# fxslava/tiny_mp2v_dec

Hardware: AMD Instinct MI355X
Metric: decoded frames/sec + GB/s vs HBM roofline, 1080p 4:2:0 @1/2/4/8 GPU; bit-exact YUV (higher is better)
Workload: dtype u8

## Files before the change

### tiny_mp2v_dec_amd/csrc/recon.hip

```cpp
#include <hip/hip_runtime.h>

#include <cstdlib>
#include <stdint.h>
#include <stdlib.h>

#include "recon_kernel.h"

namespace mp2vg {

typedef short short2_t __attribute__((ext_vector_type(2)));

__device__ __forceinline__ short2_t adds2(short2_t a, short2_t b) { return __builtin_elementwise_add_sat(a, b); }
__device__ __forceinline__ short2_t subs2(short2_t a, short2_t b) { return __builtin_elementwise_sub_sat(a, b); }
__device__ __forceinline__ short2_t shl2(short2_t a, int n) {
    return __builtin_bit_cast(short2_t, __builtin_bit_cast(ushort2, a) << (unsigned short)n);
}
__device__ __forceinline__ short2_t mulhi2(short2_t a, int c) {
    const uint32_t u = __builtin_bit_cast(uint32_t, a);
    const int lo = (int)(short)(u & 0xffffu) * c, hi = ((int)u >> 16) * c;
    return __builtin_bit_cast(short2_t, __builtin_amdgcn_perm((uint32_t)hi, (uint32_t)lo, 0x07060302u));
}
__device__ __forceinline__ short2_t mulhi2_x2(short2_t a, int c) {
    const short2_t h = mulhi2(a, 2 * c);
    return __builtin_bit_cast(short2_t, __builtin_bit_cast(uint32_t, h) & 0xfffefffeu);
// ... 137 lines not shown
    static constexpr int SIZE = 256 + 2 * F::CW * F::CH;
#ifndef MP2VG_RES_PAD
#define MP2VG_RES_PAD 0
#endif
    static constexpr int MBS = SIZE + MP2VG_RES_PAD;
    __device__ static constexpr int base(int plane) { return plane == 0 ? 0 : 256 + (plane - 1) * F::CW * F::CH; }
    __device__ static constexpr int width(int plane) { return plane == 0 ? 16 : F::CW; }
    __device__ static int pos(int x) { return (x & ~3) | ((x & 1) << 1) | ((x >> 1) & 1); }
};

template <class T>
__device__ __forceinline__ T gsel(const T (&v)[3], int plane) {
    return plane == 0 ? v[0] : (plane == 1 ? v[1] : v[2]);
}

#ifndef MP2VG_REC_NT
#define MP2VG_REC_NT 0
#endif
__device__ __forceinline__ uint32_t ld_rec(const uint32_t* p) {
    if (MP2VG_REC_NT) return __builtin_nontemporal_load(p);
    return *p;
}
__device__ __forceinline__ uint32_t rec_load(const uint32_t* __restrict__ mbrec, uint32_t g, uint32_t mb_last, int lane) {
    const uint32_t mb = min(g + (uint32_t)(lane & 3), mb_last);
    return ld_rec(&mbrec[(size_t)mb * 8 + ((lane >> 2) & 7)]);
}
__device__ __forceinline__ uint32_t rec_get(uint32_t rv, int f, int k) {
    return (uint32_t)__builtin_amdgcn_ds_bpermute((f * 4 + k) * 4, (int)rv);
}
template <int F, int K>
// ... 17 lines not shown

template <int NB, int K>
__device__ __forceinline__ void group_mb(Group& S, uint32_t rv, int ng, int& sb, int& cr) {
    const uint32_t r1 = rec_uni<1, K>(rv), r2 = rec_uni<2, K>(rv);
    const bool live = K < ng;
    const uint32_t cbpk = live ? ((r1 >> 16) & ((1u << NB) - 1)) : 0u;
    S.fl8 |= (live ? (r1 & 0xff) : (uint32_t)MP2VG_MB_INTRA) << (8 * K);
    S.qs8 |= (r2 & 0xff) << (8 * K);
    S.sb8 |= (uint32_t)sb << (8 * K);
    if (K == 0) S.cbp01 = cbpk;
    if (K == 1) S.cbp01 |= cbpk << 16;
    if (K == 2) S.cbp23 = cbpk;
    if (K == 3) S.cbp23 |= cbpk << 16;
    sb += __builtin_popcount(cbpk);
    cr += live ? (int)(r2 >> 16) : 0;
}

template <int NB>
__device__ __forceinline__ Group group_state(uint32_t rv, int ng) {
    Group S;
    S.fl8 = S.qs8 = S.sb8 = 0;
    int sb = 0, cr = 0;
    group_mb<NB, 0>(S, rv, ng, sb, cr);
    group_mb<NB, 1>(S, rv, ng, sb, cr);
    group_mb<NB, 2>(S, rv, ng, sb, cr);
    group_mb<NB, 3>(S, rv, ng, sb, cr);
    S.nslots = sb;
    S.ncoef = cr;
    S.coef0 = rec_uni<3, 0>(rv);
    return S;
// ... 177 lines not shown
};
__device__ __forceinline__ LaneRec lane_rec(uint32_t rv, int lane) {
    LaneRec L;
    const int k = lane & 3;
    L.r0 = rec_get(rv, 0, k);
    L.r1 = rec_get(rv, 1, k);
    const int r = (L.r1 & MP2VG_MB_FIELD_MC) ? ((lane >> 2) & 1) : 0;
    L.mvf = rec_get(rv, 4 + 2 * r, k);
    L.mvb = rec_get(rv, 5 + 2 * r, k);
    return L;
}

template <int CF, int MCM, int J, int NW, int ABL = 0>
__device__ __forceinline__ void issue_pass(const LaneRec& L, bool live, int lane, const Geo& geo,
                                           __amdgpu_buffer_rsrc_t ref_fwd, __amdgpu_buffer_rsrc_t ref_bwd,
                                           Tap<NW>& tf, Tap<NW>& tb, int dir = 0) {
    using F = Fmt<CF>;
    int k, plane, py;
    pass_row<CF, J>(lane, k, plane, py);
    const uint32_t fl = L.r1 & 0xffff;
    const bool none = !live || (fl & MP2VG_MB_INTRA);
    const bool bwd = fl & MP2VG_MB_BWD;
    const bool fwd = !none && (MCM == 1 || (fl & MP2VG_MB_FWD) || !bwd);
    const bool field = fl & MP2VG_MB_FIELD_MC;
    const int pw = plane == 0 ? 16 : F::CW;
    const int phm = plane == 0 ? 16 : F::CH;
    const int gx = (int)(L.r0 & 0xffff) * pw;
    const int mbyb = (int)(L.r0 >> 16) * phm;
    const int r = field ? (py & 1) : 0;
    const int stride = J == 0 ? geo.stride[0] : geo.stride[1];
    const int ph = J == 0 ? geo.ph[0] : geo.ph[1];
    constexpr bool TL = J == 0 || kChromaTiles;
    const uint32_t off = (TL ? 2u : 1u) * (uint32_t)gsel(geo.plane_off, plane);
    const uint32_t mv1 = (MCM == 1 && dir) ? L.mvb : L.mvf;
    const int fsh = 8 + 2 * r + (MCM == 1 ? dir : 0);
    constexpr bool R2 = MP2VG_ROW2_LOAD && MCM == 2;
    tap_issue<CF, NW, ABL, TL, R2>(tf, fwd, ref_fwd, off, mv1, plane, gx, py, phm, mbyb, field, (fl >> fsh) & 1, stride, ph);
    if (MCM == 2)
        tap_issue<CF, NW, ABL, TL, R2>(tb, !none && bwd, ref_bwd, off, L.mvb, plane, gx, py, phm, mbyb, field,
                                       (fl >> (9 + 2 * r)) & 1, stride, ph);
}

__device__ __forceinline__ void row_store16(uint8_t* d, uint32_t a, uint32_t b, uint32_t c, uint32_t e) {
    *(uint4*)d = make_uint4(a, b, c, e);
}
// ... 41 lines not shown
            const uint4 q1 = *(const uint4*)&res[8];
            rv[4] = q1.x; rv[5] = q1.y; rv[6] = q1.z; rv[7] = q1.w;
        }
#pragma unroll
        for (int d = 0; d < NW; d++) {
            if (!(d < 2 ? cl : cr)) continue;
            const uint32_t lo = __builtin_amdgcn_perm(0u, out[d], 0x0c020c00u);
            const uint32_t hi = __builtin_amdgcn_perm(0u, out[d], 0x0c030c01u);
            const short2_t a = __builtin_bit_cast(short2_t, lo) + __builtin_bit_cast(short2_t, rv[2 * d]);
            const short2_t c = __builtin_bit_cast(short2_t, hi) + __builtin_bit_cast(short2_t, rv[2 * d + 1]);
            out[d] = __builtin_amdgcn_perm(sat_pk_u8(c), sat_pk_u8(a), 0x05010400u);
        }
    }
    const int pw = plane == 0 ? 16 : F::CW;
    const int phm = plane == 0 ? 16 : F::CH;
    const uint32_t doff = gsel(geo.plane_off, plane) + mul24_asm((r0 >> 16) * phm + py, (uint32_t)gsel(geo.stride, plane)) +
                          (r0 & 0xffff) * (uint32_t)pw;
    uint8_t* dst = dst_slot + doff;
    dst = live ? dst : wsink;
    if (ABL & 8192)
        dst = dst_slot + ((((r0 & 0xffff) + (r0 >> 16) * 128u) * 3u + (uint32_t)J) * 1024u + (uint32_t)lane * 16u) %
                             (uint32_t)(geo.plane_off[1] - 1024);
    if (tiles) {
        uint8_t* img = (uint8_t*)(s_res_wave + k * RL::MBS + RL::base(plane) + py * RL::width(plane));
        if (NW == 4)
            *(uint4*)img = make_uint4(out[0], out[1], out[2], out[3]);
        else
            *(uint2*)img = make_uint2(out[0], out[1]);
    }
    if (ABL & 8) {
        asm volatile("" ::"v"(out[0]), "v"(out[1]), "v"(out[2]), "v"(out[3]), "v"(dst));
// ... 11 lines not shown
        row_store8(dst, out[0], out[1]);
    }
}

template <int CF, int J, int NW>
__device__ __forceinline__ void store_pass_put8(uint32_t r0, bool live, int lane, const Geo& geo, uint8_t* wsink,
                                                uint8_t* dst_slot, __amdgpu_buffer_rsrc_t dst_rsrc,
                                                const uint8_t* res8_wave) {
    using F = Fmt<CF>;
    using RL = ResLayout<CF>;
    int k, plane, py;
    pass_row<CF, J>(lane, k, plane, py);
    const uint8_t* row = &res8_wave[k * RL::SIZE + RL::base(plane) + py * RL::width(plane)];
    const int pw = plane == 0 ? 16 : F::CW;
    const int phm = plane == 0 ? 16 : F::CH;
    const uint32_t doff = gsel(geo.plane_off, plane) + mul24_asm((r0 >> 16) * phm + py, (uint32_t)gsel(geo.stride, plane)) +
                          (r0 & 0xffff) * (uint32_t)pw;
    uint8_t* dst = live ? dst_slot + doff : wsink;
    if (NW == 4) {
        const uint4 q = *(const uint4*)row;
        const uint4 o = make_uint4(__builtin_amdgcn_perm(q.x, q.x, 0x03010200u), __builtin_amdgcn_perm(q.y, q.y, 0x03010200u),
                                   __builtin_amdgcn_perm(q.z, q.z, 0x03010200u), __builtin_amdgcn_perm(q.w, q.w, 0x03010200u));
        if (MP2VG_ROW_POL != 0)
            pol_store16<MP2VG_ROW_POL>(dst_rsrc, live ? doff : kNoTap, o);
        else
            row_store16(dst, o.x, o.y, o.z, o.w);
    } else {
        const uint2 q = *(const uint2*)row;
        const uint2 o = make_uint2(__builtin_amdgcn_perm(q.x, q.x, 0x03010200u), __builtin_amdgcn_perm(q.y, q.y, 0x03010200u));
        if (MP2VG_ROW_POL != 0)
            pol_store8<MP2VG_ROW_POL>(dst_rsrc, live ? doff : kNoTap, o);
// ... 13 lines not shown
    const uint4 q = *(const uint4*)img_row<CF, NAT>(img, k, plane, py);
    return make_uint4(unswz(q.x, NAT), unswz(q.y, NAT), unswz(q.z, NAT), unswz(q.w, NAT));
}
template <int CF, bool NAT>
__device__ __forceinline__ uint2 img_row8(const uint8_t* img, int k, int plane, int py) {
    const uint2 q = *(const uint2*)img_row<CF, NAT>(img, k, plane, py);
    return make_uint2(unswz(q.x, NAT), unswz(q.y, NAT));
}
template <int CF, bool NAT, int ABL = 0>
__device__ __forceinline__ void tile_group(uint32_t mx0, uint32_t mby, int lane, const Geo& geo, uint8_t* wsink,
                                           uint8_t* dst_tiles, __amdgpu_buffer_rsrc_t tile_rsrc, const uint8_t* res8) {
    using F = Fmt<CF>;
    constexpr bool POL = MP2VG_TILE_POL != 0;
    for (int plane = 0; plane < (CF == 3 && kChromaTiles ? 3 : 1); plane++) {
        uint8_t* tp = dst_tiles + 2u * gsel(geo.plane_off, plane);
        const uint32_t ncol = (uint32_t)gsel(geo.stride, plane) >> 4;
#pragma nounroll
        for (int i = 0; i < 2; i++) {
            const int u = lane + 64 * i;
            int j, r, h;
            if (u < 96) {
                j = u >> 5, r = ((u >> 3) & 3) * 4 + ((u & 7) >> 1), h = u & 1;
            } else {
                const int side = (u - 96) >> 4;
                r = u & 15, h = side, j = side ? -1 : 3;
            }
            const uint4 v = img_row16<CF, NAT>(res8, j + h, plane, r);
            const bool none = j < 0 && mx0 == 0;
            const uint32_t o = tile_row<16>(mx0 + (uint32_t)j, mby * 16u + (uint32_t)r, ncol) + (uint32_t)h * 16u;
            if (POL)
                pol_store16<MP2VG_TILE_POL>(tile_rsrc, none ? kNoTap : 2u * gsel(geo.plane_off, plane) + o, v);
// ... 116 lines not shown
        pa = (lds_uint4_t*)(uintptr_t)(b0 + (uint32_t)(ca << 4));
        pb = (lds_uint4_t*)(uintptr_t)(b0 + (uint32_t)(cb << 4));
    }
}
__device__ __forceinline__ void put8_rows(uint32_t a0, uint32_t step, const short2_t (&s)[8]) {
#pragma unroll
    for (int y = 0; y < 8; y++) *(lds_u16_t*)(uintptr_t)(a0 + (uint32_t)y * step) = (uint16_t)sat_pk_u8(s[y] >> (short)6);
}

struct SliceCtx {
    const uint32_t* mbrec;
    const uint32_t* coefs;
    uint8_t* dst_slot;
    uint8_t* dst_tiles;
    __amdgpu_buffer_rsrc_t dst_rsrc, tile_rsrc;
    bool tiles;
    int dir;
    uint8_t* wsink;
    __amdgpu_buffer_rsrc_t ref_fwd, ref_bwd;
    __amdgpu_buffer_rsrc_t cref_fwd, cref_bwd;
    __amdgpu_buffer_rsrc_t coef_rsrc;
    uint32_t mb_begin, mb_end;
    uint32_t wpos, step;
    int half;
};

template <int CF>
__device__ __forceinline__ uint32_t dq_entry(const Group& S, int lane) {
    constexpr int NB = Fmt<CF>::NB;
    const int k = lane >> 4, bb = lane & 15;
    const uint32_t cbpk = pick16(S.cbp01, S.cbp23, k);
    const bool coded = bb < NB && ((cbpk >> bb) & 1);
    const uint32_t slot = pick8(S.sb8, k) + (uint32_t)__builtin_popcount(cbpk & ((1u << bb) - 1));
    const uint32_t intra = pick8(S.fl8, k) & MP2VG_MB_INTRA;
    const uint32_t wsel = (bb < 6 ? 0u : 2u) + (intra ? 0u : 1u);
    return (slot & 0xff) | (pick8(S.qs8, k) << 8) | (wsel << 16) | (intra << 18) | ((uint32_t)coded << 19);
}

__device__ __forceinline__ int mul24i_asm(int a, int b) {
    int r;
    asm("v_mul_i32_i24 %0, %1, %2" : "=v"(r) : "v"(a), "v"(b));
    return r;
}

template <class LT, bool INTRA_ONLY = false, int NB = 6>
__device__ __forceinline__ void dequant_word(LT& L, int wave, uint32_t w, uint32_t qs8, bool live = true, int h = 0,
                                             int buf = 0) {
    if constexpr (INTRA_ONLY) {
        const uint32_t k = (w >> 26) & 3u, b = (w >> 22) & 15u;
        const int slot = (int)(k * NB + b);
// ... 102 lines not shown
    if (g >= mb_end) return;
    const int kl = lane & 3;

    Tap<4> t0f, t0b;
    Tap<NWC> t1f, t1b;
    Tap<NWC> t2f, t2b;
    Group S;
    constexpr int NCW = MCM == 0 ? (CF == 3 ? 24 : (CF == 2 ? 12 : 8)) : 2;
    uint32_t gr0, gr1, rvN, cw[NCW];
    bool glive;
    {
        const uint32_t rv = rec_load(c.mbrec, g, mb_last, lane);
        const int ng = (int)min(mb_end - g, (uint32_t)G);
        glive = kl < ng;
        const LaneRec R = lane_rec(rv, lane);
        if (MCM) issue_pass<CF, MCM, 0, 4, ABL>(R, glive, lane, geo, c.ref_fwd, c.ref_bwd, t0f, t0b, c.dir);
        S = group_state<NB>(rv, ng);
        gr0 = R.r0;
        gr1 = R.r1;
        __builtin_amdgcn_sched_barrier(0);
        rvN = rec_load(c.mbrec, g + STEP < mb_end ? g + STEP : g, mb_last, lane);
        prefetch_words<MCM, NCW>(cw, c, S.coef0, S.ncoef, lane);
        __builtin_amdgcn_sched_barrier(0);
        if (MCM) {
            issue_pass<CF, MCM, 1, NWC, ABL>(R, glive, lane, geo, c.cref_fwd, c.cref_bwd, t1f, t1b, c.dir);
            if (CF != 1) issue_pass<CF, MCM, 2, NWC, ABL>(R, glive, lane, geo, c.cref_fwd, c.cref_bwd, t2f, t2b, c.dir);
        }
        __builtin_amdgcn_sched_barrier(0);
        if (!(ABL & 8)) {
#pragma unroll
            for (int j = 0; j < Passes<CF>::N; j++) ((uint32_t*)c.wsink)[j * 4] = 0u;
        }
    }

    Stamps st;
#pragma unroll
    for (int i = 0; i < 7; i++) st.acc[i] = 0;
    stamp<ABL>(st, -1);
    for (; g < mb_end; g += STEP) {
        stamp<ABL>(st, 6);
        uint32_t p0[4] = {0, 0, 0, 0}, p1[NWC], p2[NWC];
// ... 2 lines not shown
        if (MCM) {
            touch(t0f), touch(t1f);
            if (MCM == 2) touch(t0b), touch(t1b);
            if (CF != 1) touch(t2f);
            if (CF != 1 && MCM == 2) touch(t2b);
            predict<MCM, 4, ABL>(t0f, t0b, lane, p0);
            predict<MCM, NWC, ABL>(t1f, t1b, lane, p1);
            if (CF != 1) predict<MCM, NWC, ABL>(t2f, t2b, lane, p2);
        }

        stamp<ABL>(st, 0);
        const uint32_t gn = g + STEP < mb_end ? g + STEP : g;
        const int ngN = (int)min(mb_end - gn, (uint32_t)G);
        const bool gliveN = kl < ngN;
        const LaneRec R = lane_rec(rvN, lane);
        if (MCM) issue_pass<CF, MCM, 0, 4, ABL>(R, gliveN, lane, geo, c.ref_fwd, c.ref_bwd, t0f, t0b, c.dir);
        const Group SN = group_state<NB>(rvN, ngN);
        __builtin_amdgcn_sched_barrier(0);
        rvN = rec_load(c.mbrec, g + 2 * STEP < mb_end ? g + 2 * STEP : g, mb_last, lane);

        stamp<ABL>(st, 1);
        if constexpr (MCM != 0) {
            const uint32_t e = dq_entry<CF>(S, lane);
            L.dq[wave][lane] = e;
            if (e & (1u << 19)) L.map[wave][e & 0xff] = (uint8_t)lane;
            wave_sync();
        }
        if (!(ABL & 4)) {
            if constexpr (MCM == 0) {
#pragma unroll
                for (int j = 0; j < NCW; j++) {
                    if (64 * j >= S.ncoef) break;
                    dequant_word<LT, true, NB>(L, wave, cw[j], S.qs8, 64 * j + lane < S.ncoef, c.half);
                }
            } else {
#pragma unroll
                for (int j = 0; j < NCW; j++)
                    if (64 * j + lane < S.ncoef) dequant_word<LT, false, NB>(L, wave, cw[j], S.qs8, true, c.half);
            }
            constexpr int XW = MCM == 0 ? 8 : 2;
// ... 34 lines not shown
                if (v == 0 && intra) par ^= ra.x & 1u;
                par = (par ^ (par >> 16)) & 1u;
                par ^= (uint32_t)__builtin_amdgcn_ds_swizzle((int)par, 0x041F);
                par ^= (uint32_t)__builtin_amdgcn_ds_swizzle((int)par, 0x081F);
                if (v == 6) rb.w ^= (par ^ 1u) << 16;
                short2_t s[8] = {__builtin_bit_cast(short2_t, ra.x), __builtin_bit_cast(short2_t, ra.y),
                                 __builtin_bit_cast(short2_t, ra.z), __builtin_bit_cast(short2_t, ra.w),
                                 __builtin_bit_cast(short2_t, rb.x), __builtin_bit_cast(short2_t, rb.y),
                                 __builtin_bit_cast(short2_t, rb.z), __builtin_bit_cast(short2_t, rb.w)};
                idct_1d<true>(s);
                pass1_store<LT>(bw, slot, v, s);
            }
            wave_sync();
            __builtin_amdgcn_sched_barrier(0);
            if (MCM) {
                issue_pass<CF, MCM, 1, NWC, ABL>(R, gliveN, lane, geo, c.cref_fwd, c.cref_bwd, t1f, t1b, c.dir);
                if (CF != 1) issue_pass<CF, MCM, 2, NWC, ABL>(R, gliveN, lane, geo, c.cref_fwd, c.cref_bwd, t2f, t2b, c.dir);
            }
            __builtin_amdgcn_sched_barrier(0);
            stamp<ABL>(st, 3);
            for (int t = lane; t < (((ABL & 1) || ((ABL & (131072 | 262144)) && odd)) ? 0 : S.nslots * 4); t += 64) {
                const int slot = t >> 2, xq = t & 3;
                const int x = (xq & 1) | ((xq & 2) << 1);
                short* const bw = (short*)L.blk[wave];
                lds_uint4_t *pa, *pb;
                slot_chunks<LT>(bw, slot, x, x + 2, pa, pb);
                const uint4 ra = ld16(pa);
                const uint4 rb = ld16(pb);
                zero16(pa);
                zero16(pb);
                short2_t s[8];
                interleave(ra, rb, s);
// ... 64 lines not shown
                        int plane, x0, y0, ys;
                        block_origin<CF>(bb, dctf, plane, x0, y0, ys);
                        const int rw = RL::width(plane);
                        const int xp = RL::pos(x0 + x);
                        const uint32_t a0 = (uint32_t)(uintptr_t)(lds_u16_t*)((uint8_t*)L.res[wave] + RL::base(plane)) +
                                            mul24_asm((uint32_t)k, (uint32_t)RL::SIZE) + (uint32_t)(y0 * rw + xp);
                        put8_rows(a0, (uint32_t)(ys * rw), sv);
                    }
                }
                wave_sync();
            }
            stamp<ABL>(st, 3);
        }

        stamp<ABL>(st, 4);
        if constexpr (LT::COMPACT) {
            const uint8_t* res8 = (const uint8_t*)L.res[wave];
            store_pass_put8<CF, 0, 4>(gr0, glive, lane, geo, c.wsink, c.dst_slot, c.dst_rsrc, res8);
            store_pass_put8<CF, 1, NWC>(gr0, glive, lane, geo, c.wsink, c.dst_slot, c.dst_rsrc, res8);
            if (CF != 1) store_pass_put8<CF, 2, NWC>(gr0, glive, lane, geo, c.wsink, c.dst_slot, c.dst_rsrc, res8);
            if (TILES && c.tiles) {
                const uint32_t r00 = (uint32_t)__builtin_amdgcn_readfirstlane((int)gr0);
                tile_group<CF, false, ABL>(r00 & 0xffff, r00 >> 16, lane, geo, c.wsink, c.dst_tiles, c.tile_rsrc, res8);
            }
        } else {
            store_pass<CF, 0, 4, ABL>(gr0, gr1, glive, lane, geo, c.wsink, c.dst_slot, c.dst_rsrc, MCM != 2 && c.tiles, L.res[wave], p0);
            store_pass<CF, 1, NWC, ABL>(gr0, gr1, glive, lane, geo, c.wsink, c.dst_slot, c.dst_rsrc, MCM != 2 && c.tiles, L.res[wave], p1);
            if (CF != 1) store_pass<CF, 2, NWC, ABL>(gr0, gr1, glive, lane, geo, c.wsink, c.dst_slot, c.dst_rsrc, MCM != 2 && c.tiles, L.res[wave], p2);
            if (MCM != 2 && c.tiles) {
                wave_sync();
                const uint32_t r00 = (uint32_t)__builtin_amdgcn_readfirstlane((int)gr0);
                tile_group<CF, true, ABL>(r00 & 0xffff, r00 >> 16, lane, geo, c.wsink, c.dst_tiles, c.tile_rsrc,
                                          (const uint8_t*)L.res[wave]);
            }
        }
        wave_sync();

        stamp<ABL>(st, 5);
        S = SN;
        gr0 = R.r0;
        gr1 = R.r1;
        glive = gliveN;
    }
    if ((ABL & 16) && lane == 0) {
        unsigned long long* out = (unsigned long long*)(geo.sink + 1024) + 8 * MCM;
#pragma unroll
        for (int i = 0; i < 7; i++) atomicAdd(&out[i], (unsigned long long)st.acc[i]);
        atomicAdd(&out[7], 1ull);
    }
}

template <int CF, int MCM, int ABL = 0>
__global__ __launch_bounds__((64 * kernel_waves<MCM, ABL>())) __attribute__((amdgpu_waves_per_eu((MCM == 0 || MCM == 4) && (ABL & ~kAblCompact) == 0 ? (CF == 3 ? 4 : 6) : (CF == 3 ? 3 : 4)))) void recon_kernel(const mp2vg_picture_t* __restrict__ pics,
                                                    const uint32_t* __restrict__ mbrec,
                                                    const uint32_t* __restrict__ coefs,
                                                    const SliceDesc* __restrict__ slices,
                                                    const Geo geo,
                                                    const uint32_t slice_base, const uint32_t nslices,
                                                    const uint32_t mates) {
    using LT = Lds<CF, compact_layout<MCM, ABL>(), kernel_waves<MCM, ABL>()>;
    __shared__ __attribute__((aligned(128))) LT L;
    const int tid = threadIdx.x;
    const int lane = tid & 63;
    const int wave = __builtin_amdgcn_readfirstlane(tid >> 6);
    static_assert(slices_per_wg<CF, MCM, ABL>(4) <= (uint32_t)LT::NH, "one matrix set per slice");
    const uint32_t spw = slices_per_wg<CF, MCM, ABL>(mates);
    const bool two = spw > 1;
    const uint32_t wps = 4u / spw;
    const uint32_t nunits = (nslices + spw - 1) / spw;
    const uint32_t b = blockIdx.x, q8 = nunits / 8, r8 = nunits % 8, xcd = b % 8;
    const uint32_t unit = xcd * q8 + min(xcd, r8) + b / 8;
    const int half = two ? (int)((uint32_t)wave / wps) : 0;
    const uint32_t si = spw * unit + (uint32_t)half;
    const bool have = si < nslices;
    const SliceDesc sd = slices[slice_base + min(si, nslices - 1)];
    const mp2vg_picture_t* pic = pics + sd.pic;
// ... 6 lines not shown
        L.scan[64 * half + lane] = (uint8_t)(LT::WB ? 2 * pos : pos);
        if constexpr (LT::WB && MP2VG_I_KBTAB) {
            const int k = lane >> 4, bb = lane & 15;
            const uint32_t slot = (uint32_t)(k * Fmt<CF>::NB + (bb < Fmt<CF>::NB ? bb : 0));
            L.kbtab[lane] = (((slot << 7) | ((slot << 4) & 0x70u)) << 8) | ((uint32_t)k * 8u);
        }
        if constexpr (LT::WB && CF != 1) {
#pragma unroll
            for (int bb = 0; bb < Fmt<CF>::NB; bb++) L.Wb[bb][lane] = pic->W[bb < 6 ? 0 : 2][lane];
        }
    }
    for (int i = lane; i < LT::NBUF * LT::MAXS * LT::BLK / 2; i += 64) ((uint32_t*)L.blk[wave * LT::NBUF])[i] = 0;
    __syncthreads();
    if (!have) return;

    SliceCtx c;
    c.mbrec = mbrec;
    c.coefs = coefs;
    c.dst_slot = (uint8_t*)geo.ftab[pic->dst_slot];
    c.wsink = geo.sink + 2048 + ((b * LT::NWAVES + wave) & 1023) * 64;
    c.dst_tiles = (uint8_t*)geo.ttab[pic->dst_slot];
    c.dst_rsrc = slot_rsrc(c.dst_slot, (uint32_t)geo.slot_bytes);
    c.tile_rsrc = slot_rsrc(c.dst_tiles, (uint32_t)(2 * geo.slot_bytes));
    c.tiles = sd.reserved & 1u;
    const bool one_dir = sd.reserved & 2u;
    c.dir = (sd.reserved >> 2) & 1u;
    const int fs0 = pic->fwd_slot < 0 ? pic->dst_slot : pic->fwd_slot;
    const int bs = pic->bwd_slot < 0 ? pic->dst_slot : pic->bwd_slot;
    const int fs = c.dir ? bs : fs0;
    c.ref_fwd = slot_rsrc((const uint8_t*)geo.ttab[fs], (uint32_t)(2 * geo.slot_bytes));
    c.ref_bwd = slot_rsrc((const uint8_t*)geo.ttab[bs], (uint32_t)(2 * geo.slot_bytes));
    if (kChromaTiles) {
        c.cref_fwd = c.ref_fwd, c.cref_bwd = c.ref_bwd;
    } else {
        c.cref_fwd = slot_rsrc((const uint8_t*)geo.ftab[fs], (uint32_t)geo.slot_bytes);
        c.cref_bwd = slot_rsrc((const uint8_t*)geo.ftab[bs], (uint32_t)geo.slot_bytes);
    }
    c.coef_rsrc = __builtin_amdgcn_make_buffer_rsrc((void*)coefs, (short)0, (int)kNoTap, 0x00020000);
    c.mb_begin = sd.mb_begin;
    c.mb_end = sd.mb_begin + sd.mb_count;
    c.half = half;
    c.wpos = two ? (uint32_t)wave % wps : (uint32_t)wave;
    c.step = (two ? wps : (uint32_t)LT::NWAVES) * G;
    if constexpr (MCM == 4) {
        run_slice<CF, 0, ABL, LT, false>(c, geo, L, lane, wave);
    } else if constexpr (MCM < 3) {
        run_slice<CF, (ABL & 2) ? 0 : MCM, ABL, LT>(c, geo, L, lane, wave);
    } else {
        const int pct = pic->picture_coding_type;
        if (pct == 3 && !one_dir)
            run_slice<CF, (ABL & 2) ? 0 : 2, ABL, LT>(c, geo, L, lane, wave);
        else if (pct == 2 || one_dir)
            run_slice<CF, (ABL & 2) ? 0 : 1, ABL, LT>(c, geo, L, lane, wave);
        else
            run_slice<CF, 0, ABL, LT>(c, geo, L, lane, wave);
    }
}
__device__ __forceinline__ uint64_t mix64(uint64_t z) {
    z = (z ^ (z >> 30)) * 0xBF58476D1CE4E5B9ull;
    z = (z ^ (z >> 27)) * 0x94D049BB133111EBull;
    return z ^ (z >> 31);
}

__global__ void digest_kernel(const uint64_t* __restrict__ ftab, const int32_t* __restrict__ slots,
                              uint64_t o0, uint64_t o1, uint64_t o2, int s0, int s1, int w0, int w1, int h0, int h1,
                              unsigned long long* __restrict__ out) {
    const int si = blockIdx.y;
    const uint8_t* base = (const uint8_t*)ftab[slots[si]];
    const int rows = h0 + 2 * h1;
    uint64_t acc = 0;
    for (int row = blockIdx.x; row < rows; row += gridDim.x) {
// ... 9 lines not shown
            p = base + o2 + (uint64_t)(row - h0 - h1) * s1;
            w = w1;
        }
        for (int x = threadIdx.x * 4; x < w; x += blockDim.x * 4) {
            const uint32_t d = *(const uint32_t*)(p + x);
            acc += mix64(mix64(((uint64_t)row << 32) | (uint64_t)x) ^ (uint64_t)d);
        }
    }
    for (int off = 32; off > 0; off >>= 1) acc += __shfl_xor(acc, off);
    if ((threadIdx.x & 63) == 0) atomicAdd(&out[si], (unsigned long long)acc);
}

template <int CF, int MCM, int ABL>
static void launch_one(const KArgs& a, const Geo& g, hipStream_t stream) {
    const uint32_t spw = slices_per_wg<CF, MCM, ABL>(a.mates);
    hipLaunchKernelGGL((recon_kernel<CF, MCM, ABL>), dim3((a.nslices + spw - 1) / spw),
                       dim3(64 * kernel_waves<MCM, ABL>()), 0, stream, a.pics, (const uint32_t*)a.mbs, a.coefs,
                       a.slices, g, a.slice_base, a.nslices, spw);
}

template <int CF, int ABL>
static hipError_t launch_mcm(int mcm, const KArgs& a, const Geo& g, hipStream_t stream) {
    switch (mcm) {
    case 0: launch_one<CF, 0, ABL>(a, g, stream); break;
    case 1: launch_one<CF, 1, ABL>(a, g, stream); break;
    case 2: launch_one<CF, 2, ABL>(a, g, stream); break;
    case 3: launch_one<CF, 3, ABL>(a, g, stream); break;
    case 4: launch_one<CF, 4, ABL>(a, g, stream); break;
    default: return hipErrorInvalidValue;
    }
    return hipGetLastError();
}

hipError_t launch_recon(int cf, int mcm, const KArgs& a, hipStream_t stream) {
    Geo g;
    g.sink = a.sink;
    g.slot_bytes = a.slot_bytes;
    g.ftab = a.ftab;
    g.ttab = a.ttab;
    for (int i = 0; i < 3; i++) {
        g.plane_off[i] = (uint32_t)a.plane_off[i];
        g.stride[i] = a.stride[i];
        g.ph[i] = a.ph[i];
    }
    static const int ablate = getenv("MP2VG_ABLATE") ? atoi(getenv("MP2VG_ABLATE")) : 0;
#ifndef MP2VG_DEV_ABLATIONS
    if (ablate) return hipErrorNotSupported;
#else
    if (cf == 3 && ablate == 16) return launch_mcm<3, 16>(mcm, a, g, stream);
    if (cf == 1 && ablate) {
        switch (ablate) {
        case 1: return launch_mcm<1, 1>(mcm, a, g, stream);
        case 2: return launch_mcm<1, 2>(mcm, a, g, stream);
        case 4: return launch_mcm<1, 4>(mcm, a, g, stream);
        case 8: return launch_mcm<1, 8>(mcm, a, g, stream);
        case 15: return launch_mcm<1, 15>(mcm, a, g, stream);
        case 16: return launch_mcm<1, 16>(mcm, a, g, stream);
        case 32: return launch_mcm<1, 32>(mcm, a, g, stream);
        case 64: return launch_mcm<1, 64>(mcm, a, g, stream);
// ... 205 lines not shown
```

### tiny_mp2v_dec_amd/csrc/recon_kernel.h

```cpp
#pragma once
#include <hip/hip_runtime.h>
#include <stdint.h>

#include "../../include/mp2vg.h"

namespace mp2vg {

struct SliceDesc {
    uint32_t pic;
    uint32_t mb_begin;
    uint32_t mb_count;
    uint32_t reserved;
};

struct Launch {
    uint32_t begin, end;
    int mcm;
    int mates = 0;
    int level;
    int set;
};

struct Geo {
    uint8_t* sink;
    uint64_t slot_bytes;
    const uint64_t* ftab;
    const uint64_t* ttab;
    uint32_t plane_off[3];
    int32_t stride[3];
    int32_t ph[3];
};

struct KArgs {
    const mp2vg_picture_t* pics;
    const mp2vg_mb_t* mbs;
    const uint32_t* coefs;
    const SliceDesc* slices;
    uint8_t* sink;
    uint64_t slot_bytes;
    const uint64_t *ftab, *ttab;
    uint64_t plane_off[3];
    int32_t stride[3];
    int32_t ph[3];
    uint32_t slice_base;
    uint32_t nslices;
    uint32_t mates = 0;
};

constexpr int kFrameCopyMax = 32;
struct FrameCopy {
    const uint8_t* src[kFrameCopyMax];
    uint8_t* dst[kFrameCopyMax];
};
hipError_t launch_frame_copy(const FrameCopy& fc, int n, uint64_t bytes, hipStream_t stream);

}
```

### tiny_mp2v_dec_amd/csrc/runtime.cpp

```cpp
#include <hip/hip_runtime.h>

#include <algorithm>
#include <cstdio>
#include <cstring>
#include <string>
#include <vector>
#include <atomic>
#include <thread>

#include "export_kernel.h"
#include "hipchk.h"
#include "recon_kernel.h"
#include "syntax.h"

namespace mp2vg {
hipError_t launch_recon(int cf, int mcm, const KArgs& a, hipStream_t stream);
hipError_t launch_tile_convert(const KArgs& a, int cf, const int32_t* d_list, int n, int32_t slot0, hipStream_t stream);
hipError_t launch_clock_probe(unsigned long long* d_out, int iters, int blocks, hipStream_t stream);
hipError_t launch_block_probe(void* p, size_t bytes, int rw, int reps, void* sink, hipStream_t stream);
hipError_t launch_block_random(const void* base, size_t bytes, int waves, int iters, void* sink, hipStream_t stream);
hipError_t launch_pool_scatter(const uint64_t* tab, int nslots, uint32_t fkb, uint32_t tkb, int lock, int waves,
                               int iters, void* sink, hipStream_t stream);
hipError_t launch_digest(const uint64_t* ftab, const int32_t* d_slots, int n,
                         const uint64_t off[3], const int32_t stride[3], const int32_t w[3],
// ... 701 lines not shown
            } else if (types == 1 && slice_rows == 1 && i_split > 1 && (mbw / i_split) % 4 == 0 && mbw % i_split == 0) {
                const int pw = mbw / i_split;
                for (int r = 0; r < mbh; r++)
                    for (size_t k = i; k < j; k++)
                        for (int q = 0; q < i_split; q++)
                            slices.push_back({(uint32_t)lp[k], pics[lp[k]].mb_first + (uint32_t)(r * mbw + q * pw),
                                              (uint32_t)pw, sflags(lp[k])});
            } else {
                for (int r = 0; r < mbh; r += slice_rows)
                    for (size_t k = i; k < j; k++) push(k, r);
            }
            i = j;
        }
        l.end = (uint32_t)slices.size();
        l.mcm = types == 1 ? 0 : (types == 2 ? 1 : (types == 4 ? 2 : 3));
        static const int tilefree = dev_env("MP2VG_I_TILEFREE") ? atoi(dev_env("MP2VG_I_TILEFREE")) : 0;
        int nneed = 0;
        for (int p : lp) nneed += need[p];
        if (types == 1 && (tilefree == 2 || (tilefree && c->g.cf != 3 && nneed * 4 <= (int)lp.size()))) {
            l.mcm = 4;
            for (uint32_t k = l.begin; k < l.end; k++) slices[k].reserved = 0;
        }
        l.level = q;
        l.set = set;
        l.mates = (mates && types != 1 && l.mcm != 0 && l.mcm != 4 && mbw % 4 == 0) ? (c->g.cf == 3 ? std::min(mates, 2) : mates) : 0;
        if (tplan)
            for (int p : lp)
                if (need[p] && (pics[p].picture_coding_type == 3 || l.mcm == 4))
                    tplan->post.push_back({(int32_t)launches.size(), pics[p].dst_slot});
        launches.push_back(l);
// ... 372 lines not shown
        for (int set = 0; set < nsets; set++) {
            const int i = launch_at(set, k);
            if (i < 0) continue;
            const hipStream_t st = stream_of(set);
            if (couple == 1 && nsets > 1) {
                for (int t = 0; t < nsets; t++)
                    if (t != set && launch_at(t, k - 1) >= 0) HIPCHK(hipStreamWaitEvent(st, c->lev[launch_at(t, k - 1)], 0));
            } else if (couple == 2 && nsets > 1) {
                if (set > 0 && launch_at(set - 1, k) >= 0) HIPCHK(hipStreamWaitEvent(st, c->lev[launch_at(set - 1, k)], 0));
                if (set + 1 < nsets && launch_at(set + 1, k - 2) >= 0)
                    HIPCHK(hipStreamWaitEvent(st, c->lev[launch_at(set + 1, k - 2)], 0));
            }
            a.slice_base = launches[i].begin;
            a.nslices = launches[i].end - launches[i].begin;
            a.mates = (uint32_t)launches[i].mates;
            if (c->launch_timing) HIPCHK(hipEventRecord(H.l[2 * i], st));
            if (a.nslices) HIPCHK(launch_recon(c->g.cf, launches[i].mcm, a, st));
            {
                const auto r = b.post_of[i];
                if (r.second > r.first)
                    HIPCHK(launch_tile_convert(a, c->g.cf, b.d_post + r.first, r.second - r.first, 0, st));
            }
            if (c->launch_timing) HIPCHK(hipEventRecord(H.l[2 * i + 1], st));
            if (couple && nsets > 1) HIPCHK(hipEventRecord(c->lev[i], st));
        }
    for (int set = 0; set < nsets; set++) {
        HIPCHK(hipEventRecord(c->sev[set], stream_of(set)));
        HIPCHK(hipStreamWaitEvent(c->stream, c->sev[set], 0));
    }
    c->last_foot.assign(nsets, std::vector<uint8_t>(c->nslots, 0));
// ... 376 lines not shown
```

Measured before the change: 385,100.

## Split mixed-launch kernel by intra presence and cut scalar register pressure

Adds a separate mixed-type recon kernel that is used only when a launch contains I pictures, so the common mixed P/B kernel no longer instantiates the intra loop body. Uses asm-based rematerialization tricks (fresh_s, reloading kernel args per loop instantiation, readfirstlane for uniform bases) to keep strides, pointers and flags in SGPRs instead of holding them live across the loop. Splits group state computation into early/late parts to shorten live ranges, and simplifies dq_entry bit extraction. The intent is lower register pressure and smaller code, at the cost of extra scalar reloads and more kernel variants.

```diff
diff --git a/tiny_mp2v_dec_amd/csrc/recon.hip b/tiny_mp2v_dec_amd/csrc/recon.hip
--- a/tiny_mp2v_dec_amd/csrc/recon.hip
+++ b/tiny_mp2v_dec_amd/csrc/recon.hip
@@ -1,6 +1,8 @@
 #include <hip/hip_runtime.h>
 
+#include <cstddef>
 #include <cstdlib>
+#include <type_traits>
 #include <stdint.h>
 #include <stdlib.h>
 
@@ -175,6 +177,16 @@
     return plane == 0 ? v[0] : (plane == 1 ? v[1] : v[2]);
 }
 
+template <class T>
+__device__ __forceinline__ T fresh_s(T v, uint32_t tick) {
+    asm("" : "+s"(v) : "s"(tick));
+    return v;
+}
+
+__device__ __forceinline__ int32_t plane_stride(const Geo& geo, int plane) {
+    return plane == 0 ? geo.stride[0] : geo.stride[1];
+}
+
 #ifndef MP2VG_REC_NT
 #define MP2VG_REC_NT 0
 #endif
@@ -222,6 +234,48 @@
     if (K == 3) S.cbp23 |= cbpk << 16;
     sb += __builtin_popcount(cbpk);
     cr += live ? (int)(r2 >> 16) : 0;
+}
+
+struct GroupEarly {
+    uint32_t qs8;
+    int ncoef;
+    uint32_t coef0;
+};
+__device__ __forceinline__ GroupEarly group_early(uint32_t rv, int ng) {
+    GroupEarly E;
+    const uint32_t r2[4] = {rec_uni<2, 0>(rv), rec_uni<2, 1>(rv), rec_uni<2, 2>(rv), rec_uni<2, 3>(rv)};
+    E.qs8 = 0;
+    E.ncoef = 0;
+#pragma unroll
+    for (int k = 0; k < 4; k++) {
+        E.qs8 |= (r2[k] & 0xff) << (8 * k);
+        E.ncoef += k < ng ? (int)(r2[k] >> 16) : 0;
+    }
+    E.coef0 = rec_uni<3, 0>(rv);
+    return E;
+}
+template <int NB>
+__device__ __forceinline__ Group group_late(const GroupEarly& E, uint32_t r1_lanes, int ng) {
+    Group S;
+    S.fl8 = S.sb8 = 0;
+    S.cbp01 = S.cbp23 = 0;
+    int sb = 0;
+#pragma unroll
+    for (int k = 0; k < 4; k++) {
+        const uint32_t r1 = (uint32_t)__builtin_amdgcn_readlane((int)r1_lanes, k);
+        const bool live = k < ng;
+        const uint32_t cbpk = live ? ((r1 >> 16) & ((1u << NB) - 1)) : 0u;
+        S.fl8 |= (live ? (r1 & 0xff) : (uint32_t)MP2VG_MB_INTRA) << (8 * k);
+        S.sb8 |= (uint32_t)sb << (8 * k);
+        if (k < 2) S.cbp01 |= cbpk << (16 * k);
+        else S.cbp23 |= cbpk << (16 * (k - 2));
+        sb += __builtin_popcount(cbpk);
+    }
+    S.nslots = sb;
+    S.qs8 = E.qs8;
+    S.ncoef = E.ncoef;
+    S.coef0 = E.coef0;
+    return S;
 }
 
 template <int NB>
@@ -429,7 +483,7 @@
 template <int CF, int MCM, int J, int NW, int ABL = 0>
 __device__ __forceinline__ void issue_pass(const LaneRec& L, bool live, int lane, const Geo& geo,
                                            __amdgpu_buffer_rsrc_t ref_fwd, __amdgpu_buffer_rsrc_t ref_bwd,
-                                           Tap<NW>& tf, Tap<NW>& tb, int dir = 0) {
+                                           Tap<NW>& tf, Tap<NW>& tb, int dir, uint32_t tick) {
     using F = Fmt<CF>;
     int k, plane, py;
     pass_row<CF, J>(lane, k, plane, py);
@@ -443,7 +497,7 @@
     const int gx = (int)(L.r0 & 0xffff) * pw;
     const int mbyb = (int)(L.r0 >> 16) * phm;
     const int r = field ? (py & 1) : 0;
-    const int stride = J == 0 ? geo.stride[0] : geo.stride[1];
+    const int stride = fresh_s(J == 0 ? geo.stride[0] : geo.stride[1], tick);
     const int ph = J == 0 ? geo.ph[0] : geo.ph[1];
     constexpr bool TL = J == 0 || kChromaTiles;
     const uint32_t off = (TL ? 2u : 1u) * (uint32_t)gsel(geo.plane_off, plane);
@@ -515,7 +569,7 @@
     }
     const int pw = plane == 0 ? 16 : F::CW;
     const int phm = plane == 0 ? 16 : F::CH;
-    const uint32_t doff = gsel(geo.plane_off, plane) + mul24_asm((r0 >> 16) * phm + py, (uint32_t)gsel(geo.stride, plane)) +
+    const uint32_t doff = gsel(geo.plane_off, plane) + mul24_asm((r0 >> 16) * phm + py, (uint32_t)plane_stride(geo, plane)) +
                           (r0 & 0xffff) * (uint32_t)pw;
     uint8_t* dst = dst_slot + doff;
     dst = live ? dst : wsink;
@@ -557,7 +611,7 @@
     const uint8_t* row = &res8_wave[k * RL::SIZE + RL::base(plane) + py * RL::width(plane)];
     const int pw = plane == 0 ? 16 : F::CW;
     const int phm = plane == 0 ? 16 : F::CH;
-    const uint32_t doff = gsel(geo.plane_off, plane) + mul24_asm((r0 >> 16) * phm + py, (uint32_t)gsel(geo.stride, plane)) +
+    const uint32_t doff = gsel(geo.plane_off, plane) + mul24_asm((r0 >> 16) * phm + py, (uint32_t)plane_stride(geo, plane)) +
                           (r0 & 0xffff) * (uint32_t)pw;
     uint8_t* dst = live ? dst_slot + doff : wsink;
     if (NW == 4) {
@@ -601,7 +655,7 @@
     constexpr bool POL = MP2VG_TILE_POL != 0;
     for (int plane = 0; plane < (CF == 3 && kChromaTiles ? 3 : 1); plane++) {
         uint8_t* tp = dst_tiles + 2u * gsel(geo.plane_off, plane);
-        const uint32_t ncol = (uint32_t)gsel(geo.stride, plane) >> 4;
+        const uint32_t ncol = (uint32_t)plane_stride(geo, plane) >> 4;
 #pragma nounroll
         for (int i = 0; i < 2; i++) {
             const int u = lane + 64 * i;
@@ -748,7 +802,7 @@
     uint8_t* dst_slot;
     uint8_t* dst_tiles;
     __amdgpu_buffer_rsrc_t dst_rsrc, tile_rsrc;
-    bool tiles;
+    uint32_t tiles;
     int dir;
     uint8_t* wsink;
     __amdgpu_buffer_rsrc_t ref_fwd, ref_bwd;
@@ -763,11 +817,12 @@
 __device__ __forceinline__ uint32_t dq_entry(const Group& S, int lane) {
     constexpr int NB = Fmt<CF>::NB;
     const int k = lane >> 4, bb = lane & 15;
-    const uint32_t cbpk = pick16(S.cbp01, S.cbp23, k);
-    const bool coded = bb < NB && ((cbpk >> bb) & 1);
+    const uint32_t cbpk = __builtin_amdgcn_perm(S.cbp23, S.cbp01, 0x0c0c0100u + (uint32_t)k * 0x0202u);
+    static_assert(NB <= 16, "cbp bits");
+    const bool coded = (cbpk >> bb) & 1;
     const uint32_t slot = pick8(S.sb8, k) + (uint32_t)__builtin_popcount(cbpk & ((1u << bb) - 1));
     const uint32_t intra = pick8(S.fl8, k) & MP2VG_MB_INTRA;
-    const uint32_t wsel = (bb < 6 ? 0u : 2u) + (intra ? 0u : 1u);
+    const uint32_t wsel = (((uint32_t)bb + 10u) >> 4) * 2u + (intra ? 0u : 1u);
     return (slot & 0xff) | (pick8(S.qs8, k) << 8) | (wsel << 16) | (intra << 18) | ((uint32_t)coded << 19);
 }
 
@@ -900,7 +955,7 @@
         const int ng = (int)min(mb_end - g, (uint32_t)G);
         glive = kl < ng;
         const LaneRec R = lane_rec(rv, lane);
-        if (MCM) issue_pass<CF, MCM, 0, 4, ABL>(R, glive, lane, geo, c.ref_fwd, c.ref_bwd, t0f, t0b, c.dir);
+        if (MCM) issue_pass<CF, MCM, 0, 4, ABL>(R, glive, lane, geo, c.ref_fwd, c.ref_bwd, t0f, t0b, c.dir, g);
         S = group_state<NB>(rv, ng);
         gr0 = R.r0;
         gr1 = R.r1;
@@ -909,8 +964,8 @@
         prefetch_words<MCM, NCW>(cw, c, S.coef0, S.ncoef, lane);
         __builtin_amdgcn_sched_barrier(0);
         if (MCM) {
-            issue_pass<CF, MCM, 1, NWC, ABL>(R, glive, lane, geo, c.cref_fwd, c.cref_bwd, t1f, t1b, c.dir);
-            if (CF != 1) issue_pass<CF, MCM, 2, NWC, ABL>(R, glive, lane, geo, c.cref_fwd, c.cref_bwd, t2f, t2b, c.dir);
+            issue_pass<CF, MCM, 1, NWC, ABL>(R, glive, lane, geo, c.cref_fwd, c.cref_bwd, t1f, t1b, c.dir, g);
+            if (CF != 1) issue_pass<CF, MCM, 2, NWC, ABL>(R, glive, lane, geo, c.cref_fwd, c.cref_bwd, t2f, t2b, c.dir, g);
         }
         __builtin_amdgcn_sched_barrier(0);
         if (!(ABL & 8)) {
@@ -943,16 +998,17 @@
         const int ngN = (int)min(mb_end - gn, (uint32_t)G);
         const bool gliveN = kl < ngN;
         const LaneRec R = lane_rec(rvN, lane);
-        if (MCM) issue_pass<CF, MCM, 0, 4, ABL>(R, gliveN, lane, geo, c.ref_fwd, c.ref_bwd, t0f, t0b, c.dir);
-        const Group SN = group_state<NB>(rvN, ngN);
+        if (MCM) issue_pass<CF, MCM, 0, 4, ABL>(R, gliveN, lane, geo, c.ref_fwd, c.ref_bwd, t0f, t0b, c.dir, g);
+        const GroupEarly SN = group_early(rvN, ngN);
         __builtin_amdgcn_sched_barrier(0);
-        rvN = rec_load(c.mbrec, g + 2 * STEP < mb_end ? g + 2 * STEP : g, mb_last, lane);
+        rvN = rec_load(c.mbrec, g + 2 * STEP < mb_end ? g + 2 * STEP : g, fresh_s(mb_end, g) - 1u, lane);
 
         stamp<ABL>(st, 1);
         if constexpr (MCM != 0) {
             const uint32_t e = dq_entry<CF>(S, lane);
-            L.dq[wave][lane] = e;
-            if (e & (1u << 19)) L.map[wave][e & 0xff] = (uint8_t)lane;
+            const int wc = fresh_s(wave, g);
+            L.dq[wc][lane] = e;
+            if (e & (1u << 19)) L.map[wc][e & 0xff] = (uint8_t)lane;
             wave_sync();
         }
         if (!(ABL & 4)) {
@@ -1017,8 +1073,8 @@
             wave_sync();
             __builtin_amdgcn_sched_barrier(0);
             if (MCM) {
-                issue_pass<CF, MCM, 1, NWC, ABL>(R, gliveN, lane, geo, c.cref_fwd, c.cref_bwd, t1f, t1b, c.dir);
-                if (CF != 1) issue_pass<CF, MCM, 2, NWC, ABL>(R, gliveN, lane, geo, c.cref_fwd, c.cref_bwd, t2f, t2b, c.dir);
+                issue_pass<CF, MCM, 1, NWC, ABL>(R, gliveN, lane, geo, c.cref_fwd, c.cref_bwd, t1f, t1b, c.dir, g);
+                if (CF != 1) issue_pass<CF, MCM, 2, NWC, ABL>(R, gliveN, lane, geo, c.cref_fwd, c.cref_bwd, t2f, t2b, c.dir, g);
             }
             __builtin_amdgcn_sched_barrier(0);
             stamp<ABL>(st, 3);
@@ -1113,20 +1169,21 @@
         }
 
         stamp<ABL>(st, 4);
+        const bool tiles = fresh_s(c.tiles, g) != 0u;
         if constexpr (LT::COMPACT) {
             const uint8_t* res8 = (const uint8_t*)L.res[wave];
             store_pass_put8<CF, 0, 4>(gr0, glive, lane, geo, c.wsink, c.dst_slot, c.dst_rsrc, res8);
             store_pass_put8<CF, 1, NWC>(gr0, glive, lane, geo, c.wsink, c.dst_slot, c.dst_rsrc, res8);
             if (CF != 1) store_pass_put8<CF, 2, NWC>(gr0, glive, lane, geo, c.wsink, c.dst_slot, c.dst_rsrc, res8);
-            if (TILES && c.tiles) {
+            if (TILES && tiles) {
                 const uint32_t r00 = (uint32_t)__builtin_amdgcn_readfirstlane((int)gr0);
                 tile_group<CF, false, ABL>(r00 & 0xffff, r00 >> 16, lane, geo, c.wsink, c.dst_tiles, c.tile_rsrc, res8);
             }
         } else {
-            store_pass<CF, 0, 4, ABL>(gr0, gr1, glive, lane, geo, c.wsink, c.dst_slot, c.dst_rsrc, MCM != 2 && c.tiles, L.res[wave], p0);
-            store_pass<CF, 1, NWC, ABL>(gr0, gr1, glive, lane, geo, c.wsink, c.dst_slot, c.dst_rsrc, MCM != 2 && c.tiles, L.res[wave], p1);
-            if (CF != 1) store_pass<CF, 2, NWC, ABL>(gr0, gr1, glive, lane, geo, c.wsink, c.dst_slot, c.dst_rsrc, MCM != 2 && c.tiles, L.res[wave], p2);
-            if (MCM != 2 && c.tiles) {
+            store_pass<CF, 0, 4, ABL>(gr0, gr1, glive, lane, geo, c.wsink, c.dst_slot, c.dst_rsrc, MCM != 2 && tiles, L.res[wave], p0);
+            store_pass<CF, 1, NWC, ABL>(gr0, gr1, glive, lane, geo, c.wsink, c.dst_slot, c.dst_rsrc, MCM != 2 && tiles, L.res[wave], p1);
+            if (CF != 1) store_pass<CF, 2, NWC, ABL>(gr0, gr1, glive, lane, geo, c.wsink, c.dst_slot, c.dst_rsrc, MCM != 2 && tiles, L.res[wave], p2);
+            if (MCM != 2 && tiles) {
                 wave_sync();
                 const uint32_t r00 = (uint32_t)__builtin_amdgcn_readfirstlane((int)gr0);
                 tile_group<CF, true, ABL>(r00 & 0xffff, r00 >> 16, lane, geo, c.wsink, c.dst_tiles, c.tile_rsrc,
@@ -1136,7 +1193,7 @@
         wave_sync();
 
         stamp<ABL>(st, 5);
-        S = SN;
+        S = group_late<NB>(SN, R.r1, (int)min(fresh_s(mb_end, g) - gn, (uint32_t)G));
         gr0 = R.r0;
         gr1 = R.r1;
         glive = gliveN;
@@ -1149,16 +1206,27 @@
     }
 }
 
-template <int CF, int MCM, int ABL = 0>
-__global__ __launch_bounds__((64 * kernel_waves<MCM, ABL>())) __attribute__((amdgpu_waves_per_eu((MCM == 0 || MCM == 4) && (ABL & ~kAblCompact) == 0 ? (CF == 3 ? 4 : 6) : (CF == 3 ? 3 : 4)))) void recon_kernel(const mp2vg_picture_t* __restrict__ pics,
-                                                    const uint32_t* __restrict__ mbrec,
-                                                    const uint32_t* __restrict__ coefs,
-                                                    const SliceDesc* __restrict__ slices,
-                                                    const Geo geo,
-                                                    const uint32_t slice_base, const uint32_t nslices,
-                                                    const uint32_t mates) {
-    using LT = Lds<CF, compact_layout<MCM, ABL>(), kernel_waves<MCM, ABL>()>;
-    __shared__ __attribute__((aligned(128))) LT L;
+__device__ __forceinline__ const uint8_t* uniform_base(uint64_t a) {
+    const uint32_t lo = (uint32_t)__builtin_amdgcn_readfirstlane((int)(uint32_t)a);
+    const uint32_t hi = (uint32_t)__builtin_amdgcn_readfirstlane((int)(uint32_t)(a >> 32));
+    return (const uint8_t*)(((uint64_t)hi << 32) | lo);
+}
+
+struct ReconArgs {
+    const mp2vg_picture_t* pics;
+    const uint32_t* mbrec;
+    const uint32_t* coefs;
+    const SliceDesc* slices;
+    Geo geo;
+    uint32_t slice_base, nslices, mates;
+};
+static_assert(offsetof(ReconArgs, geo) == 32 && offsetof(ReconArgs, slice_base) == 32 + sizeof(Geo), "kernel-argument layout");
+
+template <int CF, int MCM, int ABL, bool INTRA, class LT>
+__device__ __forceinline__ void recon_body(LT& L, const mp2vg_picture_t* __restrict__ pics,
+                                           const uint32_t* __restrict__ mbrec, const uint32_t* __restrict__ coefs,
+                                           const SliceDesc* __restrict__ slices, const Geo& geo,
+                                           const uint32_t slice_base, const uint32_t nslices, const uint32_t mates) {
     const int tid = threadIdx.x;
     const int lane = tid & 63;
     const int wave = __builtin_amdgcn_readfirstlane(tid >> 6);
@@ -1195,47 +1263,92 @@
     __syncthreads();
     if (!have) return;
 
-    SliceCtx c;
-    c.mbrec = mbrec;
-    c.coefs = coefs;
-    c.dst_slot = (uint8_t*)geo.ftab[pic->dst_slot];
-    c.wsink = geo.sink + 2048 + ((b * LT::NWAVES + wave) & 1023) * 64;
-    c.dst_tiles = (uint8_t*)geo.ttab[pic->dst_slot];
-    c.dst_rsrc = slot_rsrc(c.dst_slot, (uint32_t)geo.slot_bytes);
-    c.tile_rsrc = slot_rsrc(c.dst_tiles, (uint32_t)(2 * geo.slot_bytes));
-    c.tiles = sd.reserved & 1u;
-    const bool one_dir = sd.reserved & 2u;
-    c.dir = (sd.reserved >> 2) & 1u;
-    const int fs0 = pic->fwd_slot < 0 ? pic->dst_slot : pic->fwd_slot;
-    const int bs = pic->bwd_slot < 0 ? pic->dst_slot : pic->bwd_slot;
-    const int fs = c.dir ? bs : fs0;
-    c.ref_fwd = slot_rsrc((const uint8_t*)geo.ttab[fs], (uint32_t)(2 * geo.slot_bytes));
-    c.ref_bwd = slot_rsrc((const uint8_t*)geo.ttab[bs], (uint32_t)(2 * geo.slot_bytes));
-    if (kChromaTiles) {
-        c.cref_fwd = c.ref_fwd, c.cref_bwd = c.ref_bwd;
-    } else {
-        c.cref_fwd = slot_rsrc((const uint8_t*)geo.ftab[fs], (uint32_t)geo.slot_bytes);
-        c.cref_bwd = slot_rsrc((const uint8_t*)geo.ftab[bs], (uint32_t)geo.slot_bytes);
-    }
-    c.coef_rsrc = __builtin_amdgcn_make_buffer_rsrc((void*)coefs, (short)0, (int)kNoTap, 0x00020000);
-    c.mb_begin = sd.mb_begin;
-    c.mb_end = sd.mb_begin + sd.mb_count;
-    c.half = half;
-    c.wpos = two ? (uint32_t)wave % wps : (uint32_t)wave;
-    c.step = (two ? wps : (uint32_t)LT::NWAVES) * G;
+    auto run = [&](auto loop, auto tl) {
+        constexpr int M = decltype(loop)::value;
+        asm volatile("; slice set-up, loop %0" ::"i"(M));
+        Geo gl = geo;
+        const uint32_t* mbrec_l = mbrec;
+        const uint32_t* coefs_l = coefs;
+        if constexpr (MCM == 3 && CF != 3) {
+            typedef const __attribute__((address_space(4))) ReconArgs* kargs_t;
+            const kargs_t ka = fresh_s((kargs_t)__builtin_amdgcn_kernarg_segment_ptr(), (uint32_t)M);
+            gl.sink = ka->geo.sink, gl.slot_bytes = ka->geo.slot_bytes, gl.ftab = ka->geo.ftab, gl.ttab = ka->geo.ttab;
+            for (int i = 0; i < 3; i++)
+                gl.plane_off[i] = ka->geo.plane_off[i], gl.stride[i] = ka->geo.stride[i], gl.ph[i] = ka->geo.ph[i];
+            mbrec_l = ka->mbrec;
+            coefs_l = ka->coefs;
+        }
+        SliceCtx c;
+        c.mbrec = mbrec_l;
+        c.coefs = coefs_l;
+        c.dst_slot = (uint8_t*)uniform_base(gl.ftab[pic->dst_slot]);
+        c.wsink = gl.sink + 2048 + ((b * LT::NWAVES + wave) & 1023) * 64;
+        c.dst_tiles = (uint8_t*)uniform_base(gl.ttab[pic->dst_slot]);
+        c.dst_rsrc = slot_rsrc(c.dst_slot, (uint32_t)gl.slot_bytes);
+        c.tile_rsrc = slot_rsrc(c.dst_tiles, (uint32_t)(2 * gl.slot_bytes));
+        c.tiles = sd.reserved & 1u;
+        c.dir = (sd.reserved >> 2) & 1u;
+        const int fs0 = pic->fwd_slot < 0 ? pic->dst_slot : pic->fwd_slot;
+        const int bs = pic->bwd_slot < 0 ? pic->dst_slot : pic->bwd_slot;
+        const int fs = c.dir ? bs : fs0;
+        c.ref_fwd = slot_rsrc(uniform_base(gl.ttab[fs]), (uint32_t)(2 * gl.slot_bytes));
+        c.ref_bwd = slot_rsrc(uniform_base(gl.ttab[bs]), (uint32_t)(2 * gl.slot_bytes));
+        if (kChromaTiles) {
+            c.cref_fwd = c.ref_fwd, c.cref_bwd = c.ref_bwd;
+        } else {
+            c.cref_fwd = slot_rsrc(uniform_base(gl.ftab[fs]), (uint32_t)gl.slot_bytes);
+            c.cref_bwd = slot_rsrc(uniform_base(gl.ftab[bs]), (uint32_t)gl.slot_bytes);
+        }
+        c.coef_rsrc = __builtin_amdgcn_make_buffer_rsrc((void*)coefs_l, (short)0, (int)kNoTap, 0x00020000);
+        c.mb_begin = sd.mb_begin;
+        c.mb_end = sd.mb_begin + sd.mb_count;
+        c.half = half;
+        c.wpos = two ? (uint32_t)wave % wps : (uint32_t)wave;
+        c.step = (two ? wps : (uint32_t)LT::NWAVES) * G;
+        run_slice<CF, M, ABL, LT, decltype(tl)::value>(c, gl, L, lane, wave);
+    };
+    using std::integral_constant;
+    constexpr int NOMC = (ABL & 2) ? 1 : 0;
     if constexpr (MCM == 4) {
-        run_slice<CF, 0, ABL, LT, false>(c, geo, L, lane, wave);
+        run(integral_constant<int, 0>{}, integral_constant<bool, false>{});
     } else if constexpr (MCM < 3) {
-        run_slice<CF, (ABL & 2) ? 0 : MCM, ABL, LT>(c, geo, L, lane, wave);
+        run(integral_constant<int, NOMC ? 0 : MCM>{}, integral_constant<bool, true>{});
     } else {
         const int pct = pic->picture_coding_type;
+        const bool one_dir = sd.reserved & 2u;
         if (pct == 3 && !one_dir)
-            run_slice<CF, (ABL & 2) ? 0 : 2, ABL, LT>(c, geo, L, lane, wave);
+            run(integral_constant<int, NOMC ? 0 : 2>{}, integral_constant<bool, true>{});
         else if (pct == 2 || one_dir)
-            run_slice<CF, (ABL & 2) ? 0 : 1, ABL, LT>(c, geo, L, lane, wave);
-        else
-            run_slice<CF, 0, ABL, LT>(c, geo, L, lane, wave);
-    }
+            run(integral_constant<int, NOMC ? 0 : 1>{}, integral_constant<bool, true>{});
+        else if constexpr (INTRA)
+            run(integral_constant<int, 0>{}, integral_constant<bool, true>{});
+    }
+}
+
+template <int CF, int MCM, int ABL = 0>
+__global__ __launch_bounds__((64 * kernel_waves<MCM, ABL>())) __attribute__((amdgpu_waves_per_eu((MCM == 0 || MCM == 4) && (ABL & ~kAblCompact) == 0 ? (CF == 3 ? 4 : 6) : (CF == 3 ? 3 : 4)))) void recon_kernel(const mp2vg_picture_t* __restrict__ pics,
+                                                    const uint32_t* __restrict__ mbrec,
+                                                    const uint32_t* __restrict__ coefs,
+                                                    const SliceDesc* __restrict__ slices,
+                                                    const Geo geo,
+                                                    const uint32_t slice_base, const uint32_t nslices,
+                                                    const uint32_t mates) {
+    using LT = Lds<CF, compact_layout<MCM, ABL>(), kernel_waves<MCM, ABL>()>;
+    __shared__ __attribute__((aligned(128))) LT L;
+    recon_body<CF, MCM, ABL, false, LT>(L, pics, mbrec, coefs, slices, geo, slice_base, nslices, mates);
+}
+
+template <int CF, int ABL = 0>
+__global__ __launch_bounds__((64 * kernel_waves<3, ABL>())) __attribute__((amdgpu_waves_per_eu(CF == 3 ? 3 : 4))) void recon_kernel_mixed_i(const mp2vg_picture_t* __restrict__ pics,
+                                                    const uint32_t* __restrict__ mbrec,
+                                                    const uint32_t* __restrict__ coefs,
+                                                    const SliceDesc* __restrict__ slices,
+                                                    const Geo geo,
+                                                    const uint32_t slice_base, const uint32_t nslices,
+                                                    const uint32_t mates) {
+    using LT = Lds<CF, compact_layout<3, ABL>(), kernel_waves<3, ABL>()>;
+    __shared__ __attribute__((aligned(128))) LT L;
+    recon_body<CF, 3, ABL, true, LT>(L, pics, mbrec, coefs, slices, geo, slice_base, nslices, mates);
 }
 __device__ __forceinline__ uint64_t mix64(uint64_t z) {
     z = (z ^ (z >> 30)) * 0xBF58476D1CE4E5B9ull;
@@ -1275,8 +1388,15 @@
 template <int CF, int MCM, int ABL>
 static void launch_one(const KArgs& a, const Geo& g, hipStream_t stream) {
     const uint32_t spw = slices_per_wg<CF, MCM, ABL>(a.mates);
-    hipLaunchKernelGGL((recon_kernel<CF, MCM, ABL>), dim3((a.nslices + spw - 1) / spw),
-                       dim3(64 * kernel_waves<MCM, ABL>()), 0, stream, a.pics, (const uint32_t*)a.mbs, a.coefs,
+    const dim3 grid((a.nslices + spw - 1) / spw), block(64 * kernel_waves<MCM, ABL>());
+    if constexpr (MCM == 3) {
+        if (a.intra) {
+            hipLaunchKernelGGL((recon_kernel_mixed_i<CF, ABL>), grid, block, 0, stream, a.pics, (const uint32_t*)a.mbs,
+                               a.coefs, a.slices, g, a.slice_base, a.nslices, spw);
+            return;
+        }
+    }
+    hipLaunchKernelGGL((recon_kernel<CF, MCM, ABL>), grid, block, 0, stream, a.pics, (const uint32_t*)a.mbs, a.coefs,
                        a.slices, g, a.slice_base, a.nslices, spw);
 }
 
@@ -1304,6 +1424,7 @@
         g.stride[i] = a.stride[i];
         g.ph[i] = a.ph[i];
     }
+    if (g.stride[1] != g.stride[2]) return hipErrorInvalidValue;
     static const int ablate = getenv("MP2VG_ABLATE") ? atoi(getenv("MP2VG_ABLATE")) : 0;
 #ifndef MP2VG_DEV_ABLATIONS
     if (ablate) return hipErrorNotSupported;
diff --git a/tiny_mp2v_dec_amd/csrc/recon_kernel.h b/tiny_mp2v_dec_amd/csrc/recon_kernel.h
--- a/tiny_mp2v_dec_amd/csrc/recon_kernel.h
+++ b/tiny_mp2v_dec_amd/csrc/recon_kernel.h
@@ -19,6 +19,7 @@
     int mates = 0;
     int level;
     int set;
+    bool intra = false;
 };
 
 struct Geo {
@@ -45,6 +46,7 @@
     uint32_t slice_base;
     uint32_t nslices;
     uint32_t mates = 0;
+    uint32_t intra = 0;
 };
 
 constexpr int kFrameCopyMax = 32;
diff --git a/tiny_mp2v_dec_amd/csrc/runtime.cpp b/tiny_mp2v_dec_amd/csrc/runtime.cpp
--- a/tiny_mp2v_dec_amd/csrc/runtime.cpp
+++ b/tiny_mp2v_dec_amd/csrc/runtime.cpp
@@ -739,6 +739,7 @@
         }
         l.end = (uint32_t)slices.size();
         l.mcm = types == 1 ? 0 : (types == 2 ? 1 : (types == 4 ? 2 : 3));
+        l.intra = l.mcm == 3 && (types & 1);
         static const int tilefree = dev_env("MP2VG_I_TILEFREE") ? atoi(dev_env("MP2VG_I_TILEFREE")) : 0;
         int nneed = 0;
         for (int p : lp) nneed += need[p];
@@ -1141,6 +1142,7 @@
             a.slice_base = launches[i].begin;
             a.nslices = launches[i].end - launches[i].begin;
             a.mates = (uint32_t)launches[i].mates;
+            a.intra = launches[i].intra ? 1u : 0u;
             if (c->launch_timing) HIPCHK(hipEventRecord(H.l[2 * i], st));
             if (a.nslices) HIPCHK(launch_recon(c->g.cf, launches[i].mcm, a, st));
             {
```

Result: no change. 384,700 (-0.1%).
